# wwood/CoverM

Hardware: NVIDIA H100
Metric: reads/sec `coverm contig` (mean+trimmed_mean+covered_fraction) (higher is better)
Workload: dtype i32

## Files before the change

coverm_b200/csrc/cmb_decode_slices.hpp:

```cpp
#pragma once
#include <cstdint>

#ifndef __CUDACC__
#define __host__
#define __device__
#endif

constexpr uint64_t SLICE_EVENT_BYTES = 18;

inline uint64_t decode_slice_budget(uint64_t room, bool events, uint64_t events_held, uint64_t done, uint64_t total, uint64_t iv_done,
                                    double side) {
  if (done == 0 || done >= total) return room / 2;
  uint64_t reserve = 0;
  if (events) {
    const double final_list = (double)SLICE_EVENT_BYTES * (double)iv_done * ((double)total / (double)done);
    reserve = 2 * final_list > (double)events_held ? (uint64_t)(2 * final_list) - events_held : 0;
  }
  if (room <= reserve) return 0;
  return (uint64_t)((double)(room - reserve) / (1.0 + (side > 0 ? side : 0)));
}

__host__ __device__ inline uint32_t pair_cut_after(bool eligible, uint32_t tid, uint32_t last, uint32_t i) {
  return eligible && tid != last ? i + 1 : 0;
}
__host__ __device__ inline uint32_t pair_cut_at(bool eligible, uint32_t tid, uint32_t last, uint32_t after, uint32_t i, uint32_t n) {
  return eligible && tid == last && i >= after ? i : n;
}

__host__ __device__ inline bool pair_order_drop(uint32_t tid, uint32_t largest_before) { return tid < largest_before; }
```

coverm_b200/csrc/cmb_device.cu:

```cuda
#include <cuda.h>
#include <cuda_runtime.h>

#include <algorithm>
#include <climits>
#include <cstdarg>
#include <cstdio>
#include <cstdlib>
#include <cstring>
#include <atomic>
#include <chrono>
#include <condition_variable>
#include <memory>
#include <mutex>
#include <string>
#include <thread>
#include <vector>

#include <nccl.h>
#include <nvtx3/nvToolsExt.h>
#include <strings.h>
#include <unistd.h>
#include <zlib.h>

#include "../../include/coverm_b200.h"
// ... 74 lines not shown
      if (PINNED) cudaFreeHost(p);
      else cudaFree(p);
    }
    p = nullptr;
    cap = 0;
  }
  int ensure(cmb_ctx* c, size_t need, size_t alloc);
  int ensure(cmb_ctx* c, size_t n) { return ensure(c, n, n); }
  int grow_keep(cmb_ctx* c, size_t used, size_t n, cudaStream_t st);
};
template <class T>
using PinnedBuf = Buf<T, true>;

struct DevBatch {
  Buf<uint8_t> slab;
  cmb_read_batch ptr{};
};

}

struct cmb_ctx {
  int device = 0;
  cudaStream_t stream = nullptr;
  std::string err;
  cmb_device_cfg cfg{};
  int sm_count = 0;
  std::vector<PinnedBuf<uint8_t>> host_slab;
  std::vector<cmb_read_batch> host_batch;
  std::vector<DevBatch> dev_batch;
  std::vector<cudaEvent_t> batch_done;
  std::vector<bool> batch_busy;
  uint32_t n_acquired = 0;
  uint32_t next_batch = 0;
  uint32_t n_contigs = 0, tid_begin = 0, tid_end = 0, n_local = 0;
  uint64_t arena_elems = 0;
  uint32_t n_chunks = 0;
  struct Reference {
    Buf<int32_t> d_arena;
    Buf<uint32_t> d_span_bits;
    Buf<uint32_t> d_word_count, d_word_off, d_word_block_sum;
    Buf<uint32_t> d_off_span, d_len, d_chunk_first;
    Buf<int32_t> d_tail_sum, d_carry_in;
    Buf<int2> d_block_agg;
    Buf<cmb_contig_stats> d_rows;
    Buf<uint32_t> d_bins;
    Buf<uint64_t> d_bin_base, d_bin_block_sum;
    Buf<uint32_t> d_bin_hi;
    Buf<cmb_hist_pair> d_pairs;
    Buf<uint32_t> d_gene_first, d_gene_start, d_gene_end, d_gene_maxlen, d_contig_len32;
    Buf<uint8_t> d_contig_seen;
    Buf<uint32_t> d_gene_bound;
  } ref;
  Buf<uint32_t> d_counters;
  Buf<ulonglong2> d_events;
  Buf<uint16_t> d_buckets;
  uint32_t kept_range[2] = {0, 0};
  ncclComm_t comm = nullptr;
  int comm_rank = 0, comm_size = 1;
  std::shared_ptr<LocalBarrier> local_barrier;
  Buf<uint8_t> d_xchg;
  Buf<cmb_hist_pair> d_pairs_all;
  Buf<int2> d_block_minmax;
  Buf<int2> d_block_xrange;
  bool have_xrange = false;
  uint32_t block_minmax_used = 0;
  bool gene_mode = false;
  uint32_t n_ref_contigs = 0;
  uint32_t gene_tid_begin = 0, gene_tid_end = 0;
  CUtensorMap tmap{};
  bool arena_dirty = true;
  bool pool_dirty = false;
  bool clean_as_you_go = true;
  cmb_params params{};
  cmb_filter_mode mode{};
  bool have_params = false, in_sample = false, ended = false;
  cudaEvent_t ev[8]{};
  cmb_sample_timing timing{};
  std::vector<std::pair<cudaEvent_t, cudaEvent_t>> k1_events;
  uint32_t k1_events_used = 0;
  uint64_t n_records = 0, n_intervals = 0;
  struct Decode {
    Buf<uint8_t> d_comp, d_inflated;
    Buf<uint64_t> d_coff, d_ustart, d_guess, d_exit, d_rec_base, d_cig_base;
    Buf<uint32_t> d_clen, d_isize, d_status, d_nrec, d_ncig, d_dirty;
    Buf<uint8_t> d_t1_scratch;
    Buf<uint32_t> d_tickets;
    Buf<uint32_t> d_block_window;
    PinnedBuf<uint32_t> h_ones;
    Buf<uint32_t> d_cnt;
    Buf<uint64_t> d_rec_off;
    Buf<uint8_t> d_tuple_slab;
    uint32_t last_n_rec = 0, last_n_cig = 0;
    bool last_valid = false;
    Buf<uint64_t> d_pair_key;
    Buf<int32_t> d_pair_mate;
    Buf<uint32_t> d_pair_next;
    Buf<unsigned long long> d_pair_tag;
    Buf<uint32_t> d_pair_head;
    Buf<uint2> d_pair_order;
    const int32_t* last_mate = nullptr;
    bool last_mate_inverse = false;
    uint32_t last_excl_n = 0xffffffffu;
    const uint8_t* last_infl_base = nullptr;
    Buf<unsigned long long> d_filter_anchor;
    Buf<uint8_t> d_filter_role;
    Buf<uint8_t> d_filter_out;
    uint64_t filter_bytes = 0;
// ... 137 lines not shown
  c->tmap = {};
  c->gene_mode = false;
}

int alloc_arena(cmb_ctx* c) {
  auto& r = c->ref;
  if (int rc = r.d_arena.ensure(c, c->arena_elems)) return rc;
  PFN_encodeTiled encode = nullptr;
  cudaDriverEntryPointQueryResult qres;
  CU_TRY(c, cudaGetDriverEntryPoint("cuTensorMapEncodeTiled", (void**)&encode, cudaEnableDefault, &qres));
  if (!encode || qres != cudaDriverEntryPointSuccess) return fail(c, CMB_E_CUDA, "cuTensorMapEncodeTiled not available in this driver");
  cuuint64_t gdim[2] = {ROW_ELEMS, c->arena_elems / ROW_ELEMS};
  cuuint64_t gstride[1] = {ROW_ELEMS * 4};
  cuuint32_t box[2] = {ROW_ELEMS, K2_BOX_ROWS};
  cuuint32_t estr[2] = {1, 1};
  CUresult res = encode(&c->tmap, CU_TENSOR_MAP_DATA_TYPE_INT32, 2, r.d_arena.p, gdim, gstride, box, estr, CU_TENSOR_MAP_INTERLEAVE_NONE,
                        CU_TENSOR_MAP_SWIZZLE_128B, CU_TENSOR_MAP_L2_PROMOTION_L2_256B, CU_TENSOR_MAP_FLOAT_OOB_FILL_NONE);
  if (res != CUDA_SUCCESS) return fail(c, CMB_E_CUDA, "cuTensorMapEncodeTiled failed with CUresult %d", (int)res);
  return CMB_OK;
}

void print_reference_bytes(const cmb_ctx* c) {
  const auto& r = c->ref;
  const uint64_t arena = r.d_arena.bytes();
  const uint64_t bitmap = r.d_span_bits.bytes() + r.d_word_count.bytes() + r.d_word_off.bytes() + r.d_word_block_sum.bytes();
  const uint64_t chunks = r.d_chunk_first.bytes() + r.d_tail_sum.bytes() + r.d_carry_in.bytes() + r.d_block_agg.bytes();
  const uint64_t rows = r.d_rows.bytes() + r.d_off_span.bytes() + r.d_len.bytes() + r.d_bin_base.bytes() + r.d_bin_block_sum.bytes() +
                        r.d_bin_hi.bytes() + r.d_gene_first.bytes() + r.d_gene_start.bytes() + r.d_gene_end.bytes() +
                        r.d_gene_maxlen.bytes() + r.d_contig_len32.bytes() + r.d_contig_seen.bytes() + r.d_gene_bound.bytes();
  const uint64_t bins = r.d_bins.bytes(), pairs = r.d_pairs.bytes();
  fprintf(stderr, "#reference_bytes\tarena=%llu\tbitmap=%llu\tchunks=%llu\trows=%llu\tbins=%llu\tpairs=%llu\ttotal=%llu\tlayout_elems=%llu\n",
          (unsigned long long)arena, (unsigned long long)bitmap, (unsigned long long)chunks, (unsigned long long)rows,
          (unsigned long long)bins, (unsigned long long)pairs, (unsigned long long)(arena + bitmap + chunks + rows + bins + pairs),
          (unsigned long long)c->arena_elems);
}

bool k1_active(const cmb_ctx* c) { return c->n_local || (c->gene_mode && c->gene_tid_begin < c->gene_tid_end); }

int launch_k1(cmb_ctx* c, const cmb_read_batch& b, uint32_t n_records, uint32_t n_intervals, uint32_t excl_n = 0xffffffffu,
              const int32_t* mate = nullptr) {
  if (n_records == 0) return CMB_OK;
  int rc_ = CMB_OK;
  const uint32_t blocks = (n_records + K1_THREADS - 1) / K1_THREADS;
  if (c->block_minmax_used + blocks > c->d_block_minmax.cap) {
    const size_t ncap = std::max<size_t>(c->d_block_minmax.cap * 2, c->block_minmax_used + blocks + 4096);
    if (int rc = c->d_block_minmax.grow_keep(c, c->block_minmax_used, ncap, c->stream)) return rc;
    if (int rc = c->d_block_xrange.grow_keep(c, c->block_minmax_used, ncap, c->stream)) return rc;
  }
  const auto& r = c->ref;
  if (!c->gene_mode) {
    const uint64_t need = c->n_intervals + n_intervals;
    if (2 * need > 0xffffffffull)
      return fail(c, CMB_E_CAPACITY, "more than 2^31 - 1 aligned blocks in one sample; split the input across more GPUs");
    if (c->d_events.cap < need && (rc_ = c->d_events.grow_keep(c, c->n_intervals, with_slack(need), c->stream))) return rc_;
  }
  K1Args a{};
  a.tid = b.tid; a.pos = b.pos; a.flag = b.flag; a.mapq = b.mapq; a.nm_state = b.nm_state; a.nm = b.nm;
  a.l_seq = b.l_seq; a.aligned = b.aligned; a.del = b.del; a.ins = b.ins; a.iv_begin = b.iv_begin;
  a.iv_start = b.iv_start; a.iv_len = b.iv_len;
  a.n = n_records;
  a.off_span = r.d_off_span; a.len = r.d_len;
  a.n_contigs = c->gene_mode ? c->n_ref_contigs : c->n_contigs; a.tid_begin = c->tid_begin; a.tid_end = c->tid_end;
  a.seg_begin = c->tid_begin;
  if (c->gene_mode) {
    a.tid_begin = c->gene_tid_begin; a.tid_end = c->gene_tid_end;
    a.gene_first = r.d_gene_first; a.gene_start = r.d_gene_start; a.gene_end = r.d_gene_end; a.gene_maxlen = r.d_gene_maxlen;
    a.contig_len = r.d_contig_len32; a.contig_seen = r.d_contig_seen; a.kept_primary = (unsigned long long*)(c->d_counters + 8);
    a.gene_bound = r.d_gene_bound;
  }
  a.arena = r.d_arena; a.span_bits = r.d_span_bits; a.tail_sum = r.d_tail_sum; a.rows = r.d_rows;
  if (!c->gene_mode) {
    a.events = c->d_events; a.iv_base = c->n_intervals; a.n_iv = n_intervals; a.word_count = r.d_word_count;
  }
  a.block_minmax = c->d_block_minmax + c->block_minmax_used;
  a.error_flags = c->d_counters + 0;
  a.block_xrange = c->comm_size > 1 || excl_n != 0xffffffffu ? c->d_block_xrange + c->block_minmax_used : nullptr;
  a.excl_n = excl_n;
  if (a.block_xrange) c->have_xrange = true;
  a.mate = mate;
  a.p = c->params;
  a.filter_single = c->mode.filter_single_reads;
  a.filter_pairs = c->mode.filter_pairs;
  if (c->k1_events_used == c->k1_events.size()) {
    cudaEvent_t e0, e1;
    CU_TRY(c, cudaEventCreate(&e0));
    CU_TRY(c, cudaEventCreate(&e1));
    c->k1_events.emplace_back(e0, e1);
  }
  auto& ev = c->k1_events[c->k1_events_used++];
  CU_TRY(c, cudaEventRecord(ev.first, c->stream));
  k1_filter_accumulate<<<blocks, K1_THREADS, 0, c->stream>>>(a);
  CU_TRY(c, cudaGetLastError());
  CU_TRY(c, cudaEventRecord(ev.second, c->stream));
  c->block_minmax_used += blocks;
  c->n_records += n_records;
  c->n_intervals += n_intervals;
  c->timing.k1_launches += 1;
  return CMB_OK;
}

template <bool HIST, bool CLEAN, bool BUCKETS>
int k2_blocks_per_sm(cmb_ctx* c, int* occ) {
  auto kern = k2_scan_reduce<HIST, CLEAN, BUCKETS>;
  constexpr uint32_t smem = k2_smem_bytes<BUCKETS>();
  CU_TRY(c, cudaFuncSetAttribute(kern, cudaFuncAttributeMaxDynamicSharedMemorySize, (int)smem));
  *occ = 0;
  CU_TRY(c, cudaOccupancyMaxActiveBlocksPerMultiprocessor(occ, kern, (int)K2_THREADS, smem));
  if (*occ < 1) return fail(c, CMB_E_CUDA, "k2_scan_reduce does not fit on an SM");
  return CMB_OK;
}

template <bool HIST, bool CLEAN, bool BUCKETS>
int launch_k2_variant(cmb_ctx* c, const K2Args& a) {
  int occ = 0;
  if (int rc = k2_blocks_per_sm<HIST, CLEAN, BUCKETS>(c, &occ)) return rc;
  const uint32_t grid = std::min<uint32_t>((c->n_chunks + K2_WARPS - 1) / K2_WARPS, (uint32_t)(occ * c->sm_count));
  if (getenv("CMB_PIPELINE_STATS"))
    fprintf(stderr, "#k2_grid\tgrid=%u\tblocks_per_sm=%d\tsms=%d\thist=%d\tclean=%d\tbuckets=%d\twarps=%u\n", grid, occ, c->sm_count,
            (int)HIST, (int)CLEAN, (int)BUCKETS, grid * K2_WARPS);
  k2_scan_reduce<HIST, CLEAN, BUCKETS><<<grid, K2_THREADS, k2_smem_bytes<BUCKETS>(), c->stream>>>(c->tmap, a);
  CU_TRY(c, cudaGetLastError());
  return CMB_OK;
}

int ensure_pool(cmb_ctx* c, uint64_t need, uint64_t alloc) {
  auto& r = c->ref;
  if (r.d_bins.cap >= need) return CMB_OK;
  if (int rc = r.d_bins.ensure(c, need, alloc)) return rc;
  CU_TRY(c, cudaMemsetAsync(r.d_bins, 0, 4 * r.d_bins.cap, c->stream));
  return CMB_OK;
}

bool small_hist() { return getenv("CMB_TEST_SMALL_HIST") != nullptr; }

int run_end_of_sample(cmb_ctx* c) {
  const bool hist = c->params.want & (CMB_WANT_HIST | CMB_WANT_HIST_CSR);
  const bool csr = c->params.want & CMB_WANT_HIST_CSR;
  const uint32_t excl = (uint32_t)std::min<uint64_t>(c->params.contig_end_exclusion, 0x7fffffffu);
  auto& r = c->ref;
  CU_TRY(c, cudaEventRecord(c->ev[2], c->stream));
  if (c->block_minmax_used) {
    k1c_check_sorted<<<1, 1024, 0, c->stream>>>(c->d_block_minmax, c->block_minmax_used, c->d_counters + 0,
                                                c->have_xrange ? c->d_block_xrange.p : nullptr, c->d_counters + 6);
    CU_TRY(c, cudaGetLastError());
  }
  {
    K1bBins g{};
    g.len = r.d_len; g.rows = r.d_rows + c->tid_begin; g.gene_bound = c->gene_mode ? r.d_gene_bound.p : nullptr;
    g.n_seg = c->n_local; g.excl = excl; g.bin_base = r.d_bin_base; g.block_sum = r.d_bin_block_sum;
    g.n_blocks = hist ? c->n_local / K1B_BLOCK + 1 : 0;
    K1bWords wd{};
    wd.count = r.d_word_count; wd.off = r.d_word_off; wd.block_sum = r.d_word_block_sum; wd.n_words = c->n_chunks * K2_WARPS;
    wd.n_blocks = c->gene_mode ? 0 : wd.n_words / K1B_BLOCK + 1;
    const uint32_t blocks = (c->n_chunks + K1B_BLOCK - 1) / K1B_BLOCK + g.n_blocks + wd.n_blocks;
    k1b_local<<<blocks, K1B_THREADS, 0, c->stream>>>(r.d_tail_sum, r.d_chunk_first, r.d_off_span, c->n_chunks, r.d_carry_in, r.d_block_agg, g, wd);
    CU_TRY(c, cudaGetLastError());
    k1b_apply<<<blocks, K1B_THREADS, 0, c->stream>>>(r.d_tail_sum, r.d_block_agg, c->n_chunks, r.d_carry_in, g, wd);
    CU_TRY(c, cudaGetLastError());
  }
  if (!c->gene_mode) {
    const uint64_t n_events = 2 * c->n_intervals;
    if (int rc = c->d_buckets.ensure(c, n_events + 8, with_slack(n_events + 8))) return rc;
    if (c->n_intervals) {
      const uint64_t blocks = (c->n_intervals + K1E_THREADS - 1) / K1E_THREADS;
      k1e_bucket_events<<<(uint32_t)blocks, K1E_THREADS, 0, c->stream>>>(c->d_events, c->n_intervals, r.d_word_off, r.d_word_count, c->d_buckets);
      CU_TRY(c, cudaGetLastError());
      c->timing.k1_launches += 1;
    }
  }
  if (hist && !small_hist()) {
    uint64_t need = c->n_records + c->n_local + 1;
    if (c->gene_mode) {
      CU_TRY(c, cudaMemcpyAsync(&need, r.d_bin_base + c->n_local, 8, cudaMemcpyDeviceToHost, c->stream));
      CU_TRY(c, cudaStreamSynchronize(c->stream));
    }
    if (int rc = ensure_pool(c, need, with_slack(need))) return rc;
    if (csr)
      if (int rc = r.d_pairs.ensure(c, need + c->n_local, with_slack(need + c->n_local))) return rc;
  }
  K2Args a{};
  a.off_span = r.d_off_span; a.len = r.d_len; a.chunk_first = r.d_chunk_first; a.carry_in = r.d_carry_in;
  a.rows = r.d_rows; a.tid_begin = c->tid_begin; a.n_local = c->n_local; a.n_chunks = c->n_chunks; a.excl = excl;
  a.arena = r.d_arena; a.span_bits = r.d_span_bits; a.load_stats = c->d_counters + 10;
  a.word_off = r.d_word_off; a.buckets = c->d_buckets;
  a.bin_base = r.d_bin_base; a.bins = r.d_bins; a.pool_cap = r.d_bins.cap; a.bin_hi = r.d_bin_hi;
  a.error_flags = c->d_counters + 0;
  CU_TRY(c, cudaEventRecord(c->ev[3], c->stream));
  int rc;
  const bool clean = c->clean_as_you_go;
  if (!c->gene_mode) {
    if (hist) rc = clean ? launch_k2_variant<true, true, true>(c, a) : launch_k2_variant<true, false, true>(c, a);
    else rc = clean ? launch_k2_variant<false, true, true>(c, a) : launch_k2_variant<false, false, true>(c, a);
  } else {
    if (hist) rc = clean ? launch_k2_variant<true, true, false>(c, a) : launch_k2_variant<true, false, false>(c, a);
    else rc = clean ? launch_k2_variant<false, true, false>(c, a) : launch_k2_variant<false, false, false>(c, a);
  }
  if (rc) return rc;
  c->timing.k2_launches = 1;
  c->arena_dirty = !c->clean_as_you_go;
  CU_TRY(c, cudaEventRecord(c->ev[4], c->stream));
  if (hist) {
    K3Args k{};
    k.len = r.d_len; k.rows = r.d_rows;
    k.tid_begin = c->tid_begin; k.n_local = c->n_local; k.excl = excl;
    k.trim_min = c->params.trim_min; k.trim_max = c->params.trim_max;
    k.bin_base = r.d_bin_base; k.bins = r.d_bins; k.pool_cap = r.d_bins.cap; k.bin_hi = r.d_bin_hi;
    k.pairs = r.d_pairs; k.pair_count = (unsigned long long*)(c->d_counters + 4); k.pair_capacity = r.d_pairs.cap;
    k.want_csr = csr; k.all_rows = c->gene_mode ? 1u : 0u; k.error_flags = c->d_counters + 0;
    const uint32_t per_block = K3_WARPS * K3_CONTIGS_PER_WARP;
    const uint32_t grid = (c->n_local + per_block - 1) / per_block;
    k3_finalize<<<grid, K3_THREADS, 0, c->stream>>>(k);
    CU_TRY(c, cudaGetLastError());
    c->timing.k3_launches = 1;
  }
  CU_TRY(c, cudaEventRecord(c->ev[5], c->stream));
  return CMB_OK;
}

int collect_errors_and_timing(cmb_ctx* c, uint32_t* counters_out) {
  uint32_t h[13];
  CU_TRY(c, cudaMemcpyAsync(h, c->d_counters, sizeof h, cudaMemcpyDeviceToHost, c->stream));
// ... 235 lines not shown
  CU_TRY(c, cudaMemcpyAsync(r.d_gene_maxlen, maxlen.data(), 4 * n_ctg, cudaMemcpyHostToDevice, c->stream));
  CU_TRY(c, cudaMemcpyAsync(r.d_contig_len32, clen.data(), 4 * n_ctg, cudaMemcpyHostToDevice, c->stream));
  CU_TRY(c, cudaStreamSynchronize(c->stream));
  return CMB_OK;
}

int cmb_set_genes(cmb_ctx* c, uint32_t n_contigs, const uint64_t* contig_len, uint32_t n_genes, const cmb_gene* genes) {
  return set_genes(c, n_contigs, contig_len, n_genes, genes, 0, n_contigs, true);
}

int cmb_set_genes_range(cmb_ctx* c, uint32_t n_contigs, const uint64_t* contig_len, uint32_t n_genes, const cmb_gene* genes,
                        uint32_t tid_begin, uint32_t tid_end) {
  return set_genes(c, n_contigs, contig_len, n_genes, genes, tid_begin, tid_end, false);
}

int cmb_fetch_gene_extras(cmb_ctx* c, uint8_t* contig_seen, uint64_t* n_kept_primary) {
  if (!c || !contig_seen || !n_kept_primary) return fail(c, CMB_E_ARG, "cmb_fetch_gene_extras: null argument");
  if (!c->gene_mode || !c->ended) return fail(c, CMB_E_ARG, "cmb_fetch_gene_extras: no ended sample in gene mode");
  CU_TRY(c, cudaSetDevice(c->device));
  unsigned long long kp = 0;
  if (c->n_ref_contigs) CU_TRY(c, cudaMemcpyAsync(contig_seen, c->ref.d_contig_seen, c->n_ref_contigs, cudaMemcpyDeviceToHost, c->stream));
  CU_TRY(c, cudaMemcpyAsync(&kp, c->d_counters + 8, 8, cudaMemcpyDeviceToHost, c->stream));
  CU_TRY(c, cudaStreamSynchronize(c->stream));
  *n_kept_primary = kp;
  return CMB_OK;
}

int cmb_set_reference(cmb_ctx* c, uint32_t n_contigs, const uint64_t* contig_len, uint32_t tid_begin, uint32_t tid_end) {
  if (!c || !contig_len || tid_begin > tid_end || tid_end > n_contigs) return fail(c, CMB_E_ARG, "cmb_set_reference: bad arguments");
  if (c->in_sample) return fail(c, CMB_E_ARG, "cmb_set_reference: a sample is in progress");
  CU_TRY(c, cudaSetDevice(c->device));
  free_reference(c);
  c->n_contigs = n_contigs;
  c->n_ref_contigs = n_contigs;
  c->tid_begin = tid_begin;
  c->tid_end = tid_end;
  c->n_local = tid_end - tid_begin;
  std::vector<uint32_t> off_span(c->n_local + 1), len(c->n_local);
  uint64_t spans = 0;
  for (uint32_t i = 0; i < c->n_local; ++i) {
    const uint64_t L = contig_len[tid_begin + i];
    if (L > 0x7fffffffull) return fail(c, CMB_E_ARG, "cmb_set_reference: contig %u longer than 2^31-1", tid_begin + i);
    off_span[i] = (uint32_t)spans;
    len[i] = (uint32_t)L;
    spans += std::max<uint64_t>(1, (L + SPAN - 1) / SPAN);
    if (spans > CMB_MAX_SPANS)
      return fail(c, CMB_E_ARG, "cmb_set_reference: contigs [%u, %u) need more than %llu 32-base spans (about 2^37 bases), the limit of "
                  "one context; split them over more GPUs (contig shards)", tid_begin, tid_end, (unsigned long long)CMB_MAX_SPANS);
  }
  off_span[c->n_local] = (uint32_t)spans;
  const uint64_t chunks = std::max<uint64_t>(1, (spans + CHUNK_SPANS - 1) / CHUNK_SPANS);
  c->n_chunks = (uint32_t)chunks;
  c->arena_elems = chunks * CHUNK;
  std::vector<uint32_t> chunk_first(c->n_chunks + 1);
  {
    uint32_t ci = 0;
    for (uint32_t k = 0; k < c->n_chunks; ++k) {
      const uint64_t s = (uint64_t)k * CHUNK_SPANS;
      while (ci + 1 < c->n_local && off_span[ci + 1] <= s) ++ci;
      chunk_first[k] = ci;
    }
    chunk_first[c->n_chunks] = c->n_local ? c->n_local - 1 : 0;
  }
  auto& r = c->ref;
  int rc;
  if (c->n_local == 0)
    return r.d_rows.ensure(c, std::max<size_t>(1, n_contigs));
  const size_t n_words = c->arena_elems / BITMAP_ELEMS_PER_WORD;
  if ((rc = r.d_span_bits.ensure(c, n_words)) ||
      (rc = r.d_word_count.ensure(c, n_words)) || (rc = r.d_word_off.ensure(c, n_words + 1)) ||
      (rc = r.d_word_block_sum.ensure(c, n_words / K1B_BLOCK + 1)) ||
      (rc = r.d_off_span.ensure(c, (size_t)c->n_local + 1)) || (rc = r.d_len.ensure(c, c->n_local)) ||
      (rc = r.d_chunk_first.ensure(c, (size_t)c->n_chunks + 1)) || (rc = r.d_tail_sum.ensure(c, c->n_chunks)) ||
      (rc = r.d_carry_in.ensure(c, c->n_chunks)) || (rc = r.d_block_agg.ensure(c, (size_t)c->n_chunks / K1B_BLOCK + 1)) ||
      (rc = r.d_rows.ensure(c, n_contigs)))
    return rc;
  CU_TRY(c, cudaMemcpyAsync(r.d_off_span, off_span.data(), 4ull * (c->n_local + 1), cudaMemcpyHostToDevice, c->stream));
  CU_TRY(c, cudaMemcpyAsync(r.d_len, len.data(), 4ull * c->n_local, cudaMemcpyHostToDevice, c->stream));
  CU_TRY(c, cudaMemcpyAsync(r.d_chunk_first, chunk_first.data(), 4ull * (c->n_chunks + 1), cudaMemcpyHostToDevice, c->stream));
  CU_TRY(c, cudaStreamSynchronize(c->stream));
  if ((rc = r.d_bin_base.ensure(c, (size_t)c->n_local + 1)) || (rc = r.d_bin_block_sum.ensure(c, c->n_local / K1B_BLOCK + 1)) ||
      (rc = r.d_bin_hi.ensure(c, c->n_local)))
    return rc;
  CU_TRY(c, cudaMemsetAsync(r.d_bin_hi, 0, 4ull * c->n_local, c->stream));
  CU_TRY(c, cudaMemsetAsync(r.d_bin_base, 0, 8ull * (c->n_local + 1), c->stream));
  if (small_hist() && (rc = ensure_pool(c, 64, 64))) return rc;
  c->pool_dirty = false;
  c->arena_dirty = true;
  return CMB_OK;
}

int cmb_set_params(cmb_ctx* c, const cmb_params* p, cmb_filter_mode* mode_out) {
  if (!c || !p) return fail(c, CMB_E_ARG, "cmb_set_params: null argument");
  if (c->in_sample) return fail(c, CMB_E_ARG, "cmb_set_params: a sample is in progress");
  c->params = *p;
  const bool single_initial = p->min_aligned_length_single > 0 || p->min_percent_identity_single > 0.0f || p->min_aligned_percent_single > 0.0f;
  const bool pairs_initial = p->min_aligned_length_pair > 0 || p->min_percent_identity_pair > 0.0f || p->min_aligned_percent_pair > 0.0f;
  const bool fs = single_initial || (!pairs_initial && p->min_mapq != 255);
  const bool fp = pairs_initial || ((!fs || !p->include_improper_pairs) && p->min_mapq != 255);
  c->mode.filter_single_reads = p->filtering ? fs : 0;
  c->mode.filter_pairs = p->filtering ? fp : 0;
  if (mode_out) *mode_out = c->mode;
  c->have_params = true;
  return CMB_OK;
}

// ... 1310 lines not shown
    if (k && s.group) a.names = st.names;
    ks_compact<<<(uint32_t)((n_rec + 255) / 256), 256, 0, c->stream>>>(a);
    CU_TRY(c, cudaGetLastError());
    CU_TRY(c, cudaEventRecord(s.ev[1], c->stream));
    CU_TRY(c, cudaEventSynchronize(s.ev[1]));
    float ms = 0;
    cudaEventElapsedTime(&ms, s.ev[0], s.ev[1]);
    s.ms_choose += ms;
    st.n_prim = n_prim;
    st.n_iv = n_iv;
    return CMB_OK;
  };
  auto nomem = [&](const ShardBlocks& blocks, uint32_t b0, uint32_t b1, uint64_t tail) {
    return fail(c, CMB_E_NOMEM, "shard %u: not enough device memory to decode blocks %u..%u (%llu bytes); the sharded sample holds %llu bytes", k, b0, b1,
                (unsigned long long)slice_bytes(blocks, b0, b1, tail), (unsigned long long)shard_need(c, k, st.n_prim, st.n_iv));
  };
  SliceStats ss;
  const int rc = decode_in_slices(c, in, out, ss, budget, step, nomem);
  if (rc == CMB_E_DECLINED) return fail(c, CMB_E_DECLINED, "shard %u: the device decoder declined it (%s); sharded input is decoded on the device only", k, c->err.c_str());
  if (rc) return rc;
  if (getenv("CMB_PIPELINE_STATS"))
    fprintf(stderr, "#shard_slices\tshard=%u\tslices=%u\tmax_slice_bytes=%llu\tcopy_inflate_ms=%.1f\tchain_ms=%.1f\textract_ms=%.1f\tgrow_ms=%.1f\n", k,
            ss.n_slices, (unsigned long long)ss.max_slice, ss.ms_inflate, ss.ms_chain, ss.ms_extract, ms_grow);
  return CMB_OK;
}

int decode_sliced(cmb_ctx* c, const cmb_bgzf_input* in, cmb_bgzf_result* out) {
  auto& d = c->dec;
  *out = cmb_bgzf_result{};
  auto decline = [&](int rc) {
    cudaGetLastError();
    release_decode(c);
    if (int e = reset_sample(c)) return e;
    return rc;
  };
  auto room = [&]() -> uint64_t {
    if (const uint64_t lim = shard_mem_limit()) return lim;
    size_t free_b = 0, total_b = 0;
    cudaMemGetInfo(&free_b, &total_b);
    cudaGetLastError();
    return free_b + decode_bytes(c);
  };
  if (room() < SLICE_MIN_BYTES) return decline(fail(c, CMB_E_DECLINED, "cmb_submit_bgzf: not enough device memory for device-side decode"));
  uint64_t stream_end = 0;
  const uint32_t walk_end = in->ranged ? std::min(in->walk_end_block, in->n_blocks) : in->n_blocks;
  for (uint32_t b = 0; b < walk_end; ++b) stream_end += in->block_isize[b];
  const uint64_t iv0 = c->n_intervals;
  double side = 0;
  uint32_t carry = 0;
  uint64_t cut_records = 0;
  auto budget = [&](uint64_t at) -> uint64_t {
    const uint64_t done = at > in->records_at ? at - in->records_at : 0;
    const uint64_t total = stream_end > in->records_at ? stream_end - in->records_at : 0;
    return decode_slice_budget(room(), !c->gene_mode, c->d_events.bytes(), done, total, c->n_intervals - iv0, side);
  };
  auto step = [&](BgzfCall& j, cmb_bgzf_result& r, uint64_t* next) -> int {
    const uint32_t n = (uint32_t)j.n_rec;
    uint32_t n_sub = n, iv_sub = (uint32_t)j.n_cig;
    cmb_read_batch tb;
    carve_batch(d.d_tuple_slab, n, (uint32_t)j.n_cig, &tb);
    const int32_t* mate = nullptr;
    uint32_t largest = carry;
    int rc;
    if (c->mode.filter_pairs) {
      uint32_t* w = d.d_cnt + 12;
      rc = match_mates(c, d.last_infl_base, n, true, "cmb_submit_bgzf", carry, w);
      if (rc == CMB_E_NOMEM) return SLICE_HALVE;
      if (rc) return rc;
      r.n_launches += 5;
      if (j.walk_end < walk_end) {
        const uint32_t g = (n + 255) / 256;
        kd_pair_cut_after<<<g, 256, 0, c->stream>>>(d.d_pair_key, tb.tid, n, w, w + 1);
        kd_pair_cut_at<<<g, 256, 0, c->stream>>>(d.d_pair_key, tb.tid, n, w, w + 1, w + 2);
        CU_TRY(c, cudaGetLastError());
        r.n_launches += 2;
      }
      uint32_t h[3] = {0, 0, 0};
      CU_TRY(c, cudaMemcpyAsync(h, w, 12, cudaMemcpyDeviceToHost, c->stream));
      CU_TRY(c, cudaStreamSynchronize(c->stream));
      largest = h[0];
      const uint32_t cut = n - h[2];
      if (cut == 0)
        return fail(c, CMB_E_DECLINED, "cmb_submit_bgzf: the proper-pair records of reference %d do not fit in one decode slice; mates are "
                    "matched on the host", (int32_t)largest);
      if (cut < n) {
        uint64_t off = 0;
        CU_TRY(c, cudaMemcpyAsync(&off, d.d_rec_off + cut, 8, cudaMemcpyDeviceToHost, c->stream));
        CU_TRY(c, cudaMemcpyAsync(&iv_sub, tb.iv_begin + cut, 4, cudaMemcpyDeviceToHost, c->stream));
        CU_TRY(c, cudaMemsetAsync(d.d_cnt + 16, 0, 16, c->stream));
        kd_count_held<<<(n - cut + 255) / 256, 256, 0, c->stream>>>(tb.tid, tb.flag, cut, n, j.in->own_tid_begin, j.in->own_tid_end, j.in->own_unplaced,
                                                                   (unsigned long long*)(d.d_cnt + 16), (unsigned long long*)(d.d_cnt + 18));
        CU_TRY(c, cudaGetLastError());
        uint64_t held[2] = {0, 0};
        CU_TRY(c, cudaMemcpyAsync(held, d.d_cnt + 16, 16, cudaMemcpyDeviceToHost, c->stream));
        CU_TRY(c, cudaStreamSynchronize(c->stream));
        r.n_primary -= held[0];
        r.n_records -= held[1];
        r.n_intervals = iv_sub;
        r.n_launches += 1;
        *next = off;
        n_sub = cut;
        cut_records += n - cut;
      }
      mate = d.d_pair_mate;
    }
    if (k1_active(c)) {
      uint32_t excl = 0;
// ... 370 lines not shown
```

coverm_b200/csrc/cmb_k1.cuh:

```cuda
#pragma once
#include "cmb_filter_preds.cuh"
struct K1Args {
  const int32_t* tid;
  const int32_t* pos;
  const uint16_t* flag;
  const uint8_t* mapq;
  const uint8_t* nm_state;
  const uint32_t* nm;
  const uint32_t* l_seq;
  const uint32_t* aligned;
  const uint32_t* del;
  const uint32_t* ins;
  const uint32_t* iv_begin;
  const int32_t* iv_start;
  const int32_t* iv_len;
  uint32_t n;
  const uint32_t* off_span;
  const uint32_t* len;
  uint32_t n_contigs, tid_begin, tid_end, seg_begin;
  int32_t* arena;
  ulonglong2* events;
  uint64_t iv_base;
  uint32_t n_iv;
  uint32_t* word_count;
  uint32_t* span_bits;
  int32_t* tail_sum;
  cmb_contig_stats* rows;
  int2* block_minmax;
  uint32_t* error_flags;
  int2* block_xrange;
  uint32_t excl_n;
  const uint32_t* gene_first;
  const uint32_t* gene_start;
  const uint32_t* gene_end;
  const uint32_t* gene_maxlen;
  const uint32_t* contig_len;
  uint8_t* contig_seen;
  unsigned long long* kept_primary;
  uint32_t* gene_bound;
  const int32_t* mate;
  cmb_params p;
  uint8_t filter_single, filter_pairs;
};

constexpr unsigned long long K1_NO_EVENT = ~0ull;

#ifndef CMB_K1_MINBLOCKS
#define CMB_K1_MINBLOCKS 6
#endif
#ifndef CMB_K1_PREFETCH
#define CMB_K1_PREFETCH 1
#endif
__global__ void __launch_bounds__(K1_THREADS, CMB_K1_MINBLOCKS) k1_filter_accumulate(const K1Args a) {
  const uint32_t i = blockIdx.x * K1_THREADS + threadIdx.x;
  const uint32_t lane = threadIdx.x & 31, warp = threadIdx.x >> 5;
  const bool valid = i < a.n;
  const cmb_params& p = a.p;

  RecView r = {};
  int32_t tid = -1, pos = 0;
  uint32_t ins = 0, ivb = 0, ive = 0;
  if (valid) {
    tid = a.tid[i];
    pos = a.pos[i];
    r.flag = a.flag[i];
    r.mapq = a.mapq[i];
    r.nm_state = a.nm_state[i];
    r.nm = a.nm[i];
    r.l_seq = a.l_seq[i];
    r.aligned = a.aligned[i];
    r.del = a.del[i];
    ins = a.ins[i];
    ivb = a.iv_begin[i];
    ive = a.iv_begin[i + 1];
  }
#if CMB_K1_PREFETCH
  uint32_t pre_L = 0, pre_off0 = 0, pre_off1 = 0;
  int32_t pre_s = INT_MIN, pre_n = 0;
  const bool pre_seg = valid && !a.gene_first && tid >= 0 && (uint32_t)tid >= a.tid_begin && (uint32_t)tid < a.tid_end &&
                       (uint32_t)tid < a.n_contigs;
  if (pre_seg) {
    const uint32_t lc = (uint32_t)tid - a.tid_begin;
    pre_L = __ldg(a.len + lc);
    pre_off0 = __ldg(a.off_span + lc);
    pre_off1 = __ldg(a.off_span + lc + 1);
  }
  if (valid && ivb < ive) {
    pre_s = __ldg(a.iv_start + ivb);
    pre_n = __ldg(a.iv_len + ivb);
  }
#endif
  const bool unmapped = r.flag & 0x4, secondary = r.flag & 0x100, supplementary = r.flag & 0x800, proper = r.flag & 0x2;
  const bool flag_pass = !(secondary && !p.include_secondary) && !(supplementary && !p.include_supplementary) &&
                         !(!proper && !p.include_improper_pairs);
  bool keep = valid && flag_pass && !unmapped;
  bool nm_err = false;
  if (valid && p.filtering) {
    bool passes;
    if (a.filter_single && !a.filter_pairs) {
      const bool passes_filter1 = !unmapped && (p.include_supplementary || !supplementary) && (p.include_secondary || !secondary);
      passes = passes_filter1 && single_read_passes(r, p, &nm_err);
    } else {
      const int32_t mi = a.mate ? a.mate[i] : (int32_t)(i ^ 1u);
      const uint32_t m = (uint32_t)mi;
      RecView o = {};
// ... 34 lines not shown
    for (int d = 1; d < 32; d <<= 1) {
      const int o = __shfl_up_sync(FULL, pm, d);
      if ((int)lane >= d) pm = max(pm, o);
    }
    int excl = __shfl_up_sync(FULL, pm, 1);
    if (lane == 0) excl = INT_MIN;
    int kmin = keep ? tid : INT_MAX;
#pragma unroll
    for (int d = 16; d > 0; d >>= 1) kmin = min(kmin, __shfl_xor_sync(FULL, kmin, d));
    if (lane == 31) s_wmax[warp] = pm;
    if (lane == 0) s_wmin[warp] = kmin;
    __shared__ int s_xmax[K1_THREADS / 32];
    __shared__ int s_xmin[K1_THREADS / 32];
    if (a.block_xrange) {
      const bool xk = keep && i < a.excl_n;
      const int xmax = __reduce_max_sync(FULL, xk ? tid : INT_MIN);
      const int xmin = __reduce_min_sync(FULL, xk ? tid : INT_MAX);
      if (lane == 0) {
        s_xmax[warp] = xmax;
        s_xmin[warp] = xmin;
      }
    }
    __syncthreads();
    if (a.block_xrange && threadIdx.x == 0) {
      int xmax = INT_MIN, xmin = INT_MAX;
      for (uint32_t w = 0; w < K1_THREADS / 32; ++w) {
        xmax = max(xmax, s_xmax[w]);
        xmin = min(xmin, s_xmin[w]);
      }
      a.block_xrange[blockIdx.x] = make_int2(xmin, xmax);
    }
    int before = INT_MIN;
    for (uint32_t w = 0; w < warp; ++w) before = max(before, s_wmax[w]);
    if (keep && tid < max(before, excl)) err |= ERR_UNSORTED;
    if (threadIdx.x == 0) {
      int bmax = INT_MIN, bmin = INT_MAX;
      for (uint32_t w = 0; w < K1_THREADS / 32; ++w) {
        bmax = max(bmax, s_wmax[w]);
        bmin = min(bmin, s_wmin[w]);
      }
      a.block_minmax[blockIdx.x] = make_int2(bmin, bmax);
    }
  }

  auto mark_span = [&](uint64_t g) {
    const uint32_t w = (uint32_t)(g / BITMAP_ELEMS_PER_WORD);
    const uint32_t peers = __match_any_sync(__activemask(), w);
    const uint32_t bits = __reduce_or_sync(peers, 1u << ((uint32_t)(g / SPAN) % BITMAP_SPANS_PER_WORD));
    if (lane == (uint32_t)__ffs(peers) - 1) {
      atomicOr(a.span_bits + w, bits);
      if (a.word_count) atomicAdd(a.word_count + w, (uint32_t)__popc(peers));
    }
  };
  auto add_events_in = [&](uint32_t L, uint32_t off0, uint32_t off1, uint32_t s, uint64_t e) -> ulonglong2 {
    const uint64_t base = (uint64_t)off0 * SPAN;
    const uint64_t end_padded = (uint64_t)off1 * SPAN;
    const uint64_t gs = base + s;
    const bool has_end = e < L;
    ulonglong2 out = make_ulonglong2(gs << 1, K1_NO_EVENT);
    mark_span(gs);
    const uint64_t ks = gs / CHUNK;
    const bool cont_s = end_padded > (ks + 1) * (uint64_t)CHUNK;
    if (has_end) {
      const uint64_t ge = base + e;
      out.y = ge << 1 | 1u;
      mark_span(ge);
      const uint64_t ke = ge / CHUNK;
      if (ke != ks) {
        if (cont_s) atomicAdd(a.tail_sum + ks, 1);
        if (end_padded > (ke + 1) * (uint64_t)CHUNK) atomicAdd(a.tail_sum + ke, -1);
      }
    } else if (cont_s) {
      atomicAdd(a.tail_sum + ks, 1);
    }
    return out;
  };
  auto add_gene_events = [&](uint32_t lc, uint32_t s, uint64_t e) {
    const ulonglong2 ev = add_events_in(a.len[lc], a.off_span[lc], a.off_span[lc + 1], s, e);
    atomicAdd(a.arena + (ev.x >> 1), 1);
    if (ev.y != K1_NO_EVENT) atomicAdd(a.arena + (ev.y >> 1), -1);
  };

  if (a.gene_first) {
    if (keep && (uint32_t)tid - a.tid_begin < a.tid_end - a.tid_begin) {
      const bool primary = !secondary && !supplementary;
      a.contig_seen[tid] = 1;
      if (primary) atomicAdd(a.kept_primary, 1ull);
      const uint32_t CL = a.contig_len[tid];
      uint64_t ref_end = (uint32_t)pos;
      for (uint32_t k = ivb; k < ive; ++k) {
        const int32_t s = a.iv_start[k];
        if (s == INT_MIN) continue;
        if (s < 0 || (uint32_t)s >= CL) {
          err |= ERR_BOUNDS;
          continue;
        }
        ref_end = max(ref_end, (uint64_t)(uint32_t)s + (uint32_t)a.iv_len[k]);
      }
      const uint32_t g0 = a.gene_first[tid], g1 = a.gene_first[tid + 1];
      if (g0 < g1 && !(err & ERR_BOUNDS)) {
        const uint32_t maxlen = a.gene_maxlen[tid];
        const uint32_t from = (uint32_t)pos >= maxlen ? (uint32_t)pos - maxlen + 1 : 0;
        uint32_t lo = g0, hi = g1;
        while (lo < hi) {
          const uint32_t mid = (lo + hi) >> 1;
          if (a.gene_start[mid] < from) lo = mid + 1;
          else hi = mid;
        }
        const uint64_t indels = (uint64_t)ins + r.del;
        for (uint32_t g = lo; g < g1; ++g) {
          const uint32_t gsx = a.gene_start[g], gex = a.gene_end[g];
          if ((uint64_t)gsx >= max(ref_end, (uint64_t)(uint32_t)pos + 1)) break;
          const uint32_t lg = g - a.seg_begin;
          atomicAdd(a.gene_bound + lg, 1u);
          if ((uint32_t)pos >= gsx && (uint32_t)pos < gex) {
            cmb_contig_stats* row = a.rows + g;
            atomicAdd((unsigned long long*)&row->n_records, 1ull);
            if (primary) atomicAdd((unsigned long long*)&row->n_primary, 1ull);
            const uint64_t mis = r.nm >= indels ? r.nm - indels : 0;
            if (mis) atomicAdd((unsigned long long*)&row->sum_edit, (unsigned long long)mis);
            if (primary && r.aligned > 0) atomicAdd(&row->sum_identity_primary, ((double)r.aligned - (double)r.nm) / (double)r.aligned);
          }
          for (uint32_t k = ivb; k < ive; ++k) {
            const int32_t s = a.iv_start[k];
            if (s == INT_MIN) continue;
            const uint64_t e = (uint64_t)(uint32_t)s + (uint32_t)a.iv_len[k];
            if (e <= gsx || (uint32_t)s >= gex) continue;
            const uint32_t cs = max((uint32_t)s, gsx) - gsx;
            add_gene_events(lg, cs, e - gsx);
          }
        }
      }
    }
    err = __reduce_or_sync(FULL, err);
    if (err && lane == 0) atomicOr(a.error_flags, err);
    return;
  }

  const bool mine = keep && (uint32_t)tid >= a.tid_begin && (uint32_t)tid < a.tid_end;
  {
    const uint32_t mine_mask = __ballot_sync(FULL, mine);
    if (mine_mask) {
      const bool primary = !secondary && !supplementary;
      const uint32_t below = mine_mask & ((1u << lane) - 1);
      const int prev_tid = __shfl_sync(FULL, tid, below ? 31 - __clz(below) : lane);
      const uint32_t heads = __ballot_sync(FULL, mine && (!below || prev_tid != tid)) | 1u;
      const uint32_t after = heads & ~((2u << lane) - 1);
      const uint32_t run_end = after ? __ffs(after) - 1 : 32;
      const uint32_t run = (run_end == 32 ? FULL : (1u << run_end) - 1) & ~((1u << lane) - 1);
      uint64_t s_edit = mine ? r.nm : 0, s_indel = mine ? (uint64_t)ins + r.del : 0;
      double idn = 0.0;
      if (mine && r.aligned > 0) idn = ((double)r.aligned - (double)r.nm) / (double)r.aligned;
      double s_idp = primary ? idn : 0.0, s_idn = !supplementary ? idn : 0.0;
#pragma unroll
      for (uint32_t d = 1; d < 32; d <<= 1) {
        const uint64_t oe = __shfl_down_sync(FULL, s_edit, d), oi = __shfl_down_sync(FULL, s_indel, d);
        const double op = __shfl_down_sync(FULL, s_idp, d), on = __shfl_down_sync(FULL, s_idn, d);
        if (lane + d < run_end) {
          s_edit += oe;
          s_indel += oi;
          s_idp += op;
          s_idn += on;
        }
      }
      const uint32_t s_rec = __popc(mine_mask & run), s_pri = __popc(__ballot_sync(FULL, mine && primary) & run),
                     s_ns = __popc(__ballot_sync(FULL, mine && !supplementary) & run);
      if (mine && (heads >> lane & 1)) {
        cmb_contig_stats* row = a.rows + tid;
        atomicAdd((unsigned long long*)&row->n_records, (unsigned long long)s_rec);
        if (s_pri) atomicAdd((unsigned long long*)&row->n_primary, (unsigned long long)s_pri);
        if (s_ns) atomicAdd((unsigned long long*)&row->n_nonsupp, (unsigned long long)s_ns);
        if (s_edit) atomicAdd((unsigned long long*)&row->sum_edit, (unsigned long long)s_edit);
        if (s_indel) atomicAdd((unsigned long long*)&row->sum_indel, (unsigned long long)s_indel);
        if (s_idp != 0.0) atomicAdd(&row->sum_identity_primary, s_idp);
        if (s_idn != 0.0) atomicAdd(&row->sum_identity_nonsupp, s_idn);
      }
    }
  }

  if (valid) {
    const ulonglong2 none = make_ulonglong2(K1_NO_EVENT, K1_NO_EVENT);
    ulonglong2* ev = a.events + a.iv_base;
    if (i == 0)
      for (uint32_t k = 0; k < min(ivb, a.n_iv); ++k) __stcs(ev + k, none);
    if (i + 1 == a.n)
      for (uint32_t k = ive; k < a.n_iv; ++k) __stcs(ev + k, none);
    const uint32_t lc = (uint32_t)tid - a.tid_begin;
    (void)lc;
#if CMB_K1_PREFETCH
    const uint32_t L = pre_L, off0 = pre_off0, off1 = pre_off1;
#else
    uint32_t L = 0, off0 = 0, off1 = 0;
    if (mine) L = a.len[lc], off0 = a.off_span[lc], off1 = a.off_span[lc + 1];
#endif
    for (uint32_t k = ivb; k < min(ive, a.n_iv); ++k) {
      ulonglong2 out = none;
      if (mine) {
#if CMB_K1_PREFETCH
        const int32_t s = k == ivb ? pre_s : a.iv_start[k];
        const uint32_t n = (uint32_t)(k == ivb ? pre_n : a.iv_len[k]);
#else
        const int32_t s = a.iv_start[k];
        const uint32_t n = (uint32_t)a.iv_len[k];
#endif
        if (s == INT_MIN) {
        } else if (s < 0 || (uint32_t)s >= L) {
          err |= ERR_BOUNDS;
        } else {
          out = add_events_in(L, off0, off1, (uint32_t)s, (uint64_t)(uint32_t)s + n);
        }
      }
      __stcs(ev + k, out);
    }
  }
  err = __reduce_or_sync(FULL, err);
  if (err && lane == 0) atomicOr(a.error_flags, err);
}

__global__ void __launch_bounds__(1024) k1c_check_sorted(const int2* block_minmax, uint32_t n_blocks, uint32_t* error_flags,
                                                         const int2* block_xrange, uint32_t* kept_range) {
  __shared__ int s_max[1024];
  const uint32_t t = threadIdx.x;
  const uint32_t per = (n_blocks + 1023) / 1024;
  const uint32_t b0 = t * per, b1 = min(n_blocks, b0 + per);
  if (block_xrange) {
    int xmin = INT_MAX, xmax = INT_MIN;
    for (uint32_t b = b0; b < b1; ++b) {
      const int2 x = block_xrange[b];
      xmin = min(xmin, x.x);
      xmax = max(xmax, x.y);
    }
    xmin = __reduce_min_sync(FULL, xmin);
    xmax = __reduce_max_sync(FULL, xmax);
    if ((t & 31) == 0 && xmax != INT_MIN) {
      atomicMax(kept_range + 0, (uint32_t)xmax + 1u);
      atomicMax(kept_range + 1, (uint32_t)(INT_MAX - xmin));
    }
  }
  int lmax = INT_MIN;
  bool bad = false;
  for (uint32_t b = b0; b < b1; ++b) {
    const int2 mm = block_minmax[b];
    if (mm.x != INT_MAX && mm.x < lmax) bad = true;
    lmax = max(lmax, mm.y);
  }
  s_max[t] = lmax;
  __syncthreads();
  int before = INT_MIN;
  for (uint32_t k = 0; k < t; ++k) before = max(before, s_max[k]);
  for (uint32_t b = b0; b < b1 && !bad; ++b) {
    const int2 mm = block_minmax[b];
    if (mm.x != INT_MAX && mm.x < before) bad = true;
  }
  if (bad) atomicOr(error_flags, ERR_UNSORTED);
}

constexpr uint32_t K1E_THREADS = 256;
__global__ void __launch_bounds__(K1E_THREADS) k1e_bucket_events(const ulonglong2* events, uint64_t n_iv, const uint32_t* word_off,
                                                                uint32_t* word_count, uint16_t* buckets) {
  const uint64_t k = (uint64_t)blockIdx.x * K1E_THREADS + threadIdx.x;
  const uint32_t lane = threadIdx.x & 31;
  const ulonglong2 e = k < n_iv ? __ldcs(events + k) : make_ulonglong2(K1_NO_EVENT, K1_NO_EVENT);
  auto place = [&](unsigned long long x) {
    const bool has = x != K1_NO_EVENT;
    const uint32_t active = __ballot_sync(FULL, has);
    if (!has) return;
    const uint64_t g = x >> 1;
    const uint32_t w = (uint32_t)(g / BITMAP_ELEMS_PER_WORD);
    const uint32_t off = __ldg(word_off + w);
    const uint32_t peers = __match_any_sync(active, w), n = __popc(peers), head = __ffs(peers) - 1;
    uint32_t top = 0;
    if (lane == head) top = atomicSub(word_count + w, n);
    top = __shfl_sync(peers, top, head);
    const uint32_t r = top - n + __popc(peers & ((1u << lane) - 1));
    buckets[off + r] =(uint16_t)((uint32_t)(g % BITMAP_ELEMS_PER_WORD) | (uint32_t)(x & 1) << 10);
  };
  place(e.x);
  place(e.y);
}
```

Measured before the change: 5.432 billion.

## Store per-interval event entries as 32-bit offsets when arena fits

The per-interval event list was stored as two 64-bit values with the start/end flag in the low bit. It now uses two 32-bit offsets whenever the arena is under 2^32 elements, with the flag implied by the slot position. This halves event-buffer traffic in the accumulate and bucket kernels and lets the decode slice budget reserve less memory. It also replaces the serial prefix-max in the sort check with a warp-shuffle scan and restructures bucket placement to issue both match/atomic steps together. The cost is templated kernels and a runtime switch between the 32-bit and 64-bit paths.

```diff
diff --git a/coverm_b200/csrc/cmb_decode_slices.hpp b/coverm_b200/csrc/cmb_decode_slices.hpp
--- a/coverm_b200/csrc/cmb_decode_slices.hpp
+++ b/coverm_b200/csrc/cmb_decode_slices.hpp
@@ -6,14 +6,15 @@
 #define __device__
 #endif
 
-constexpr uint64_t SLICE_EVENT_BYTES = 18;
+constexpr uint64_t slice_event_bytes(uint64_t pair_bytes) { return pair_bytes + pair_bytes / 8; }
+constexpr uint64_t SLICE_EVENT_BYTES = slice_event_bytes(16);
 
 inline uint64_t decode_slice_budget(uint64_t room, bool events, uint64_t events_held, uint64_t done, uint64_t total, uint64_t iv_done,
-                                    double side) {
+                                    double side, uint64_t event_bytes = SLICE_EVENT_BYTES) {
   if (done == 0 || done >= total) return room / 2;
   uint64_t reserve = 0;
   if (events) {
-    const double final_list = (double)SLICE_EVENT_BYTES * (double)iv_done * ((double)total / (double)done);
+    const double final_list = (double)event_bytes * (double)iv_done * ((double)total / (double)done);
     reserve = 2 * final_list > (double)events_held ? (uint64_t)(2 * final_list) - events_held : 0;
   }
   if (room <= reserve) return 0;
diff --git a/coverm_b200/csrc/cmb_device.cu b/coverm_b200/csrc/cmb_device.cu
--- a/coverm_b200/csrc/cmb_device.cu
+++ b/coverm_b200/csrc/cmb_device.cu
@@ -150,7 +150,9 @@
     Buf<uint32_t> d_gene_bound;
   } ref;
   Buf<uint32_t> d_counters;
-  Buf<ulonglong2> d_events;
+  Buf<uint2> d_events;
+  bool events_u32 = true;
+  uint32_t event_units() const { return events_u32 ? 1 : 2; }
   Buf<uint16_t> d_buckets;
   uint32_t kept_range[2] = {0, 0};
   ncclComm_t comm = nullptr;
@@ -394,7 +396,8 @@
     const uint64_t need = c->n_intervals + n_intervals;
     if (2 * need > 0xffffffffull)
       return fail(c, CMB_E_CAPACITY, "more than 2^31 - 1 aligned blocks in one sample; split the input across more GPUs");
-    if (c->d_events.cap < need && (rc_ = c->d_events.grow_keep(c, c->n_intervals, with_slack(need), c->stream))) return rc_;
+    const uint32_t u = c->event_units();
+    if (c->d_events.cap < need * u && (rc_ = c->d_events.grow_keep(c, c->n_intervals * u, with_slack(need) * u, c->stream))) return rc_;
   }
   K1Args a{};
   a.tid = b.tid; a.pos = b.pos; a.flag = b.flag; a.mapq = b.mapq; a.nm_state = b.nm_state; a.nm = b.nm;
@@ -412,7 +415,7 @@
   }
   a.arena = r.d_arena; a.span_bits = r.d_span_bits; a.tail_sum = r.d_tail_sum; a.rows = r.d_rows;
   if (!c->gene_mode) {
-    a.events = c->d_events; a.iv_base = c->n_intervals; a.n_iv = n_intervals; a.word_count = r.d_word_count;
+    a.events = c->d_events.p; a.iv_base = c->n_intervals; a.n_iv = n_intervals; a.word_count = r.d_word_count;
   }
   a.block_minmax = c->d_block_minmax + c->block_minmax_used;
   a.error_flags = c->d_counters + 0;
@@ -431,7 +434,8 @@
   }
   auto& ev = c->k1_events[c->k1_events_used++];
   CU_TRY(c, cudaEventRecord(ev.first, c->stream));
-  k1_filter_accumulate<<<blocks, K1_THREADS, 0, c->stream>>>(a);
+  if (c->gene_mode || c->events_u32) k1_filter_accumulate<uint32_t><<<blocks, K1_THREADS, 0, c->stream>>>(a);
+  else k1_filter_accumulate<unsigned long long><<<blocks, K1_THREADS, 0, c->stream>>>(a);
   CU_TRY(c, cudaGetLastError());
   CU_TRY(c, cudaEventRecord(ev.second, c->stream));
   c->block_minmax_used += blocks;
@@ -505,10 +509,17 @@
     if (int rc = c->d_buckets.ensure(c, n_events + 8, with_slack(n_events + 8))) return rc;
     if (c->n_intervals) {
       const uint64_t blocks = (c->n_intervals + K1E_THREADS - 1) / K1E_THREADS;
-      k1e_bucket_events<<<(uint32_t)blocks, K1E_THREADS, 0, c->stream>>>(c->d_events, c->n_intervals, r.d_word_off, r.d_word_count, c->d_buckets);
+      if (c->events_u32)
+        k1e_bucket_events<<<(uint32_t)blocks, K1E_THREADS, 0, c->stream>>>((const K1Entries32*)c->d_events.p, c->n_intervals, r.d_word_off,
+                                                                          r.d_word_count, c->d_buckets);
+      else
+        k1e_bucket_events<<<(uint32_t)blocks, K1E_THREADS, 0, c->stream>>>((const K1Entries64*)c->d_events.p, c->n_intervals, r.d_word_off,
+                                                                          r.d_word_count, c->d_buckets);
       CU_TRY(c, cudaGetLastError());
       c->timing.k1_launches += 1;
     }
+    if (getenv("CMB_PIPELINE_STATS"))
+      fprintf(stderr, "#k1_events\tentry_bytes=%u\tslots=%llu\n", c->events_u32 ? 4u : 8u, (unsigned long long)c->n_intervals);
   }
   if (hist && !small_hist()) {
     uint64_t need = c->n_records + c->n_local + 1;
@@ -850,6 +861,7 @@
   const uint64_t chunks = std::max<uint64_t>(1, (spans + CHUNK_SPANS - 1) / CHUNK_SPANS);
   c->n_chunks = (uint32_t)chunks;
   c->arena_elems = chunks * CHUNK;
+  c->events_u32 = k1_entries_fit_u32(c->arena_elems) && !getenv("CMB_TEST_WIDE_EVENTS");
   std::vector<uint32_t> chunk_first(c->n_chunks + 1);
   {
     uint32_t ci = 0;
@@ -2266,7 +2278,8 @@
   auto budget = [&](uint64_t at) -> uint64_t {
     const uint64_t done = at > in->records_at ? at - in->records_at : 0;
     const uint64_t total = stream_end > in->records_at ? stream_end - in->records_at : 0;
-    return decode_slice_budget(room(), !c->gene_mode, c->d_events.bytes(), done, total, c->n_intervals - iv0, side);
+    return decode_slice_budget(room(), !c->gene_mode, c->d_events.bytes(), done, total, c->n_intervals - iv0, side,
+                               slice_event_bytes(8 * c->event_units()));
   };
   auto step = [&](BgzfCall& j, cmb_bgzf_result& r, uint64_t* next) -> int {
     const uint32_t n = (uint32_t)j.n_rec;
diff --git a/coverm_b200/csrc/cmb_k1.cuh b/coverm_b200/csrc/cmb_k1.cuh
--- a/coverm_b200/csrc/cmb_k1.cuh
+++ b/coverm_b200/csrc/cmb_k1.cuh
@@ -1,5 +1,6 @@
 #pragma once
 #include "cmb_filter_preds.cuh"
+#include "cmb_k1_entries.hpp"
 struct K1Args {
   const int32_t* tid;
   const int32_t* pos;
@@ -19,7 +20,7 @@
   const uint32_t* len;
   uint32_t n_contigs, tid_begin, tid_end, seg_begin;
   int32_t* arena;
-  ulonglong2* events;
+  void* events;
   uint64_t iv_base;
   uint32_t n_iv;
   uint32_t* word_count;
@@ -43,7 +44,18 @@
   uint8_t filter_single, filter_pairs;
 };
 
-constexpr unsigned long long K1_NO_EVENT = ~0ull;
+__device__ __forceinline__ void st_entries(K1Entries32* p, const K1Entries32& v) { __stcs(reinterpret_cast<uint2*>(p), make_uint2(v.x, v.y)); }
+__device__ __forceinline__ void st_entries(K1Entries64* p, const K1Entries64& v) {
+  __stcs(reinterpret_cast<ulonglong2*>(p), make_ulonglong2(v.x, v.y));
+}
+__device__ __forceinline__ K1Entries32 ld_entries(const K1Entries32* p) {
+  const uint2 v = __ldcs(reinterpret_cast<const uint2*>(p));
+  return {v.x, v.y};
+}
+__device__ __forceinline__ K1Entries64 ld_entries(const K1Entries64* p) {
+  const ulonglong2 v = __ldcs(reinterpret_cast<const ulonglong2*>(p));
+  return {v.x, v.y};
+}
 
 #ifndef CMB_K1_MINBLOCKS
 #define CMB_K1_MINBLOCKS 6
@@ -51,6 +63,7 @@
 #ifndef CMB_K1_PREFETCH
 #define CMB_K1_PREFETCH 1
 #endif
+template <class T>
 __global__ void __launch_bounds__(K1_THREADS, CMB_K1_MINBLOCKS) k1_filter_accumulate(const K1Args a) {
   const uint32_t i = blockIdx.x * K1_THREADS + threadIdx.x;
   const uint32_t lane = threadIdx.x & 31, warp = threadIdx.x >> 5;
@@ -191,18 +204,18 @@
       if (a.word_count) atomicAdd(a.word_count + w, (uint32_t)__popc(peers));
     }
   };
-  auto add_events_in = [&](uint32_t L, uint32_t off0, uint32_t off1, uint32_t s, uint64_t e) -> ulonglong2 {
+  auto add_events_in = [&](uint32_t L, uint32_t off0, uint32_t off1, uint32_t s, uint64_t e) -> K1Entries64 {
     const uint64_t base = (uint64_t)off0 * SPAN;
     const uint64_t end_padded = (uint64_t)off1 * SPAN;
     const uint64_t gs = base + s;
     const bool has_end = e < L;
-    ulonglong2 out = make_ulonglong2(gs << 1, K1_NO_EVENT);
+    K1Entries64 out = {gs, K1Entries64::NONE};
     mark_span(gs);
     const uint64_t ks = gs / CHUNK;
     const bool cont_s = end_padded > (ks + 1) * (uint64_t)CHUNK;
     if (has_end) {
       const uint64_t ge = base + e;
-      out.y = ge << 1 | 1u;
+      out.y = ge;
       mark_span(ge);
       const uint64_t ke = ge / CHUNK;
       if (ke != ks) {
@@ -215,9 +228,9 @@
     return out;
   };
   auto add_gene_events = [&](uint32_t lc, uint32_t s, uint64_t e) {
-    const ulonglong2 ev = add_events_in(a.len[lc], a.off_span[lc], a.off_span[lc + 1], s, e);
-    atomicAdd(a.arena + (ev.x >> 1), 1);
-    if (ev.y != K1_NO_EVENT) atomicAdd(a.arena + (ev.y >> 1), -1);
+    const K1Entries64 ev = add_events_in(a.len[lc], a.off_span[lc], a.off_span[lc + 1], s, e);
+    atomicAdd(a.arena + ev.x, 1);
+    if (ev.y != K1Entries64::NONE) atomicAdd(a.arena + ev.y, -1);
   };
 
   if (a.gene_first) {
@@ -318,12 +331,13 @@
   }
 
   if (valid) {
-    const ulonglong2 none = make_ulonglong2(K1_NO_EVENT, K1_NO_EVENT);
-    ulonglong2* ev = a.events + a.iv_base;
+    using E = K1Entries<T>;
+    const E none = E::none();
+    E* ev = static_cast<E*>(a.events) + a.iv_base;
     if (i == 0)
-      for (uint32_t k = 0; k < min(ivb, a.n_iv); ++k) __stcs(ev + k, none);
+      for (uint32_t k = 0; k < min(ivb, a.n_iv); ++k) st_entries(ev + k, none);
     if (i + 1 == a.n)
-      for (uint32_t k = ive; k < a.n_iv; ++k) __stcs(ev + k, none);
+      for (uint32_t k = ive; k < a.n_iv; ++k) st_entries(ev + k, none);
     const uint32_t lc = (uint32_t)tid - a.tid_begin;
     (void)lc;
 #if CMB_K1_PREFETCH
@@ -333,7 +347,7 @@
     if (mine) L = a.len[lc], off0 = a.off_span[lc], off1 = a.off_span[lc + 1];
 #endif
     for (uint32_t k = ivb; k < min(ive, a.n_iv); ++k) {
-      ulonglong2 out = none;
+      E out = none;
       if (mine) {
 #if CMB_K1_PREFETCH
         const int32_t s = k == ivb ? pre_s : a.iv_start[k];
@@ -346,10 +360,11 @@
         } else if (s < 0 || (uint32_t)s >= L) {
           err |= ERR_BOUNDS;
         } else {
-          out = add_events_in(L, off0, off1, (uint32_t)s, (uint64_t)(uint32_t)s + n);
+          const K1Entries64 g = add_events_in(L, off0, off1, (uint32_t)s, (uint64_t)(uint32_t)s + n);
+          out = {(T)g.x, (T)g.y};
         }
       }
-      __stcs(ev + k, out);
+      st_entries(ev + k, out);
     }
   }
   err = __reduce_or_sync(FULL, err);
@@ -358,7 +373,7 @@
 
 __global__ void __launch_bounds__(1024) k1c_check_sorted(const int2* block_minmax, uint32_t n_blocks, uint32_t* error_flags,
                                                          const int2* block_xrange, uint32_t* kept_range) {
-  __shared__ int s_max[1024];
+  __shared__ int s_max[64];
   const uint32_t t = threadIdx.x;
   const uint32_t per = (n_blocks + 1023) / 1024;
   const uint32_t b0 = t * per, b1 = min(n_blocks, b0 + per);
@@ -383,10 +398,28 @@
     if (mm.x != INT_MAX && mm.x < lmax) bad = true;
     lmax = max(lmax, mm.y);
   }
-  s_max[t] = lmax;
+  const uint32_t lane = t & 31, warp = t >> 5;
+  int incl = lmax;
+#pragma unroll
+  for (uint32_t d = 1; d < 32; d <<= 1) {
+    const int o = __shfl_up_sync(FULL, incl, d);
+    if (lane >= d) incl = max(incl, o);
+  }
+  int before = __shfl_up_sync(FULL, incl, 1);
+  if (lane == 0) before = INT_MIN;
+  if (lane == 31) s_max[warp] = incl;
   __syncthreads();
-  int before = INT_MIN;
-  for (uint32_t k = 0; k < t; ++k) before = max(before, s_max[k]);
+  if (warp == 0) {
+    int wi = s_max[lane];
+#pragma unroll
+    for (uint32_t d = 1; d < 32; d <<= 1) {
+      const int o = __shfl_up_sync(FULL, wi, d);
+      if (lane >= d) wi = max(wi, o);
+    }
+    s_max[32 + lane] = wi;
+  }
+  __syncthreads();
+  if (warp) before = max(before, s_max[32 + warp - 1]);
   for (uint32_t b = b0; b < b1 && !bad; ++b) {
     const int2 mm = block_minmax[b];
     if (mm.x != INT_MAX && mm.x < before) bad = true;
@@ -395,25 +428,25 @@
 }
 
 constexpr uint32_t K1E_THREADS = 256;
-__global__ void __launch_bounds__(K1E_THREADS) k1e_bucket_events(const ulonglong2* events, uint64_t n_iv, const uint32_t* word_off,
+template <class T>
+__global__ void __launch_bounds__(K1E_THREADS) k1e_bucket_events(const K1Entries<T>* events, uint64_t n_iv, const uint32_t* word_off,
                                                                 uint32_t* word_count, uint16_t* buckets) {
+  using E = K1Entries<T>;
   const uint64_t k = (uint64_t)blockIdx.x * K1E_THREADS + threadIdx.x;
   const uint32_t lane = threadIdx.x & 31;
-  const ulonglong2 e = k < n_iv ? __ldcs(events + k) : make_ulonglong2(K1_NO_EVENT, K1_NO_EVENT);
-  auto place = [&](unsigned long long x) {
-    const bool has = x != K1_NO_EVENT;
-    const uint32_t active = __ballot_sync(FULL, has);
-    if (!has) return;
-    const uint64_t g = x >> 1;
-    const uint32_t w = (uint32_t)(g / BITMAP_ELEMS_PER_WORD);
-    const uint32_t off = __ldg(word_off + w);
-    const uint32_t peers = __match_any_sync(active, w), n = __popc(peers), head = __ffs(peers) - 1;
-    uint32_t top = 0;
-    if (lane == head) top = atomicSub(word_count + w, n);
-    top = __shfl_sync(peers, top, head);
-    const uint32_t r = top - n + __popc(peers & ((1u << lane) - 1));
-    buckets[off + r] =(uint16_t)((uint32_t)(g % BITMAP_ELEMS_PER_WORD) | (uint32_t)(x & 1) << 10);
-  };
-  place(e.x);
-  place(e.y);
-}
+  const E e = k < n_iv ? ld_entries(events + k) : E::none();
+  const bool hx = e.x != E::NONE, hy = e.y != E::NONE;
+  const uint32_t wx = hx ? (uint32_t)((uint64_t)e.x / BITMAP_ELEMS_PER_WORD) : FULL;
+  const uint32_t wy = hy ? (uint32_t)((uint64_t)e.y / BITMAP_ELEMS_PER_WORD) : FULL;
+  const uint32_t px = __match_any_sync(FULL, wx), py = __match_any_sync(FULL, wy);
+  const uint32_t hdx = __ffs(px) - 1, hdy = __ffs(py) - 1;
+  uint32_t tx = 0, ty = 0;
+  if (hx && lane == hdx) tx = atomicSub(word_count + wx, (uint32_t)__popc(px));
+  if (hy && lane == hdy) ty = atomicSub(word_count + wy, (uint32_t)__popc(py));
+  const uint32_t ox = hx ? __ldg(word_off + wx) : 0, oy = hy ? __ldg(word_off + wy) : 0;
+  tx = __shfl_sync(FULL, tx, hdx);
+  ty = __shfl_sync(FULL, ty, hdy);
+  const uint32_t below = (1u << lane) - 1;
+  if (hx) buckets[ox + tx - __popc(px) + __popc(px & below)] = (uint16_t)((uint64_t)e.x % BITMAP_ELEMS_PER_WORD);
+  if (hy) buckets[oy + ty - __popc(py) + __popc(py & below)] = (uint16_t)((uint64_t)e.y % BITMAP_ELEMS_PER_WORD | 1u << 10);
+}
diff --git a/coverm_b200/csrc/cmb_k1_entries.hpp b/coverm_b200/csrc/cmb_k1_entries.hpp
--- /dev/null
+++ b/coverm_b200/csrc/cmb_k1_entries.hpp
@@ -0,0 +1,20 @@
+#pragma once
+#include <cstdint>
+
+#ifndef __CUDACC__
+#define __host__
+#define __device__
+#define __forceinline__ inline
+#endif
+
+template <class T>
+struct alignas(2 * sizeof(T)) K1Entries {
+  T x, y;
+  static constexpr T NONE = (T)~(T)0;
+  __host__ __device__ __forceinline__ static K1Entries none() { return {NONE, NONE}; }
+};
+using K1Entries32 = K1Entries<uint32_t>;
+using K1Entries64 = K1Entries<unsigned long long>;
+static_assert(sizeof(K1Entries32) == 8 && sizeof(K1Entries64) == 16, "entry pairs are stored as one 8-B / 16-B word");
+
+__host__ __device__ __forceinline__ bool k1_entries_fit_u32(uint64_t n_elems) { return n_elems <= 0xffffffffull; }
```

New measurement: 5.556 billion (median of 6 runs). Within noise of the previous version (+2.3%).
